# manospits/parallel_heat

Hardware: AMD Instinct MI355X
Metric: Mcells/sec (whole node) + sec/1000 iters, 8192^2 grid at 1/2/4/8 MI355X (higher is better)
Workload: dtype fp32; 1 GPU; model=heat2d 5-point Jacobi (fixed boundary), grid=8192x8192, global_batch=1, seq_len=67108864, parallelism=domain-decomp 1x1 (local), tb_depth 12, halo 12, schedule sync, converge_check=False

## Files before the change

### csrc/include/heat/kernels.hpp

```cpp
#pragma once

#include <hip/hip_runtime.h>

#include <cstdint>
#include <vector>

#include "heat/topology.hpp"

namespace heat::gpu {

struct StencilGeom {
  int64_t pitch = 0;
  int64_t gx0 = 0, gy0 = 0;
  int64_t nx = 0, ny = 0;
  float cx = 0.1f, cy = 0.1f;
  int numerics = 0;
  const unsigned* gate = nullptr;
};

namespace tbv {
enum : int {
  kRing3 = 0,
  kRing4 = 1,
  kRing2 = 2,
  kRamp = 3,
  kPipeMask = 3,
  kScalar = 4,
  kPrefetch6 = 8,
  kXcdGroups = 16,
  kAltDirection = 32,
  kFloat2 = 64,
  kForceAgePairs = 256,
  kDiagNoStore = 1024,
  kSplit = 2048,
  kDiagCachedRows = 4096,
  kNoAgePairs = 16384,
  kLinear = 32768,
  kNoLinear = 65536,
  kTile = 131072,
  kTileDpp = 262144,
  kShiftMixed = 524288,
  kDefault = kRamp | kScalar | kXcdGroups,
  kDefaultDeep = kDefault | kSplit,
};
}

constexpr int kTbMaxDepth = 8;
constexpr double kTbAgeRatio = 1.0;
constexpr double kTbSplitAgeWeights[2] = {1.7, 1.0};
constexpr double kTbLinearAgeWeights[4] = {2.0, 1.95, 1.15, 1.0};
constexpr int kTbDeepDepth = 12;
bool tb_depth_supported(int k);
int tb_strip_width(int k, int lane_cols = 4);
int tb_lane_cols(int variant);

void init_field(float* origin, const Layout& L, int64_t gx0, int64_t gy0, int64_t nx,
                int64_t ny, int mode, uint64_t seed, hipStream_t st);

void naive_step(const float* src, float* dst, const StencilGeom& g, const Box& box,
                unsigned* resid, hipStream_t st);

void lds_step(const float* src, float* dst, const StencilGeom& g, const Box& box,
              unsigned* resid, hipStream_t st);

void mfma_step(const float* src, float* dst, const StencilGeom& g, const Box& box,
               unsigned* resid, hipStream_t st);

struct TbChain {
  int passes = 1;
  unsigned* flags = nullptr;
  unsigned* done = nullptr;
  unsigned* err = nullptr;
  int max_units = 0;
  bool chained = false;
};
void tb_step(const float* src, float* dst, const StencilGeom& g, const Box* boxes, int nbox,
             int depth, unsigned* resid, hipStream_t st, int waves_target = 0, int variant = -1,
             int res_level = 0, TbChain* chain = nullptr);
struct TbResidentBuffers {
  float* base[2] = {nullptr, nullptr};
  int64_t origin = 0;
  int64_t bytes = 0;
  unsigned* flags = nullptr;
  int max_tiles = 0;
  unsigned* done = nullptr;
  unsigned* err = nullptr;
};
struct TbResidentCheck {
  int pass = 0, step = 0;
};
constexpr int kTbResidentMaxChecks = 64;
bool tb_resident_fits(const Box& box, int depth, int variant = -1);
void tb_resident_step(const float* src, float* dst, const StencilGeom& g, const Box& box,
                      int depth, int passes, const TbResidentBuffers& xb, hipStream_t st,
                      int variant = -1, const TbResidentCheck* checks = nullptr,
                      int nchecks = 0, unsigned* resids = nullptr, int64_t own_rows = 0,
                      int64_t own_cols = 0);

bool tb_mid_residual(int depth);
int tb_default_variant(int depth);
int tb_auto_variant(int depth, int64_t strip_rows_per_simd);
void tb_set_stamps(unsigned long long* buf, int64_t waves);
int tb_variant_lag(int variant);
bool tb_variant_deep(int variant);
bool tb_variant_split(int variant);
struct TbTuning {
  int variant = -1;
  int rounds = 0;
  int min_len = 0;
  int waves = 0;
  double edge_frac = 1.0;
  std::vector<double> age_weights;
  int tile_rows = 0;
  int tile_waves = 0;
  int tile_xl = -1;
  int tile_max_srps = 64;
  int nt = -1;
  int res_diag = 0;
};
TbTuning tb_tuning();
void tb_set_tuning(const TbTuning& t);
int tb_default_rounds();
int tb_resident_waves(int depth, int variant);
int tb_simd_count();
int tb_auto_waves_per_simd(int depth, int64_t strip_rows_per_simd, int max_per_simd);

void pack_box(const float* origin, int64_t pitch, const Box& box, float* buf, hipStream_t st);
constexpr int kMaxBoxCopies = 8;
struct BoxCopy {
  Box box;
  float* buf = nullptr;
};
void copy_boxes(float* origin, int64_t pitch, const BoxCopy* copies, int n, bool to_buf,
                hipStream_t st);
void unpack_box(const float* buf, float* origin, int64_t pitch, const Box& box, hipStream_t st);

struct DeviceChecksum {
  unsigned long long hash;
  double sum;
  int min_key, max_key;
  unsigned long long count;
};
void checksum_block(const float* origin, int64_t pitch, int64_t lx, int64_t ly, int64_t ox,
                    int64_t oy, int64_t ny, DeviceChecksum* out, hipStream_t st);
float checksum_key_to_float(int key);

struct DeviceGate {
  unsigned stop;
  unsigned reason;
  unsigned stop_check;
  unsigned checks;
  unsigned last_bits;
  unsigned pad[3];
};
void judge_check(unsigned* resid, DeviceGate* gate, double eps, bool mpi_compat, hipStream_t st,
                 int n = 1, int slots = 1, int stride = 0);
constexpr int kTbResidentSlots = 64;

void residual_box(const float* a, const float* b, int64_t pitch, const Box& box, unsigned* resid,
                  hipStream_t st);

}
```

### csrc/kernels/exp_register.hip

```cpp
#include "tb_exp.hpp"

namespace {
const heat::gpu::TbExpKernels* table() {
  using namespace heat::gpu;
  static const TbExpKernels k{&tbp::launch,          &tbp::occupancy,
                              &tbn::launch,          &tbn::occupancy,
                              &tbxm::launch_split,   &tbxm::occupancy_split,
                              &tbxnp::launch_split,  &tbc::occupancy_chain,
                              &tbc::launch_chain};
  return &k;
}
struct Register {
  Register() { heat_register_exp_kernels(table()); }
} reg;
}

extern "C" void heat_exp_register(void) { heat_register_exp_kernels(table()); }
```

### csrc/kernels/stencil.hip

```cpp
#include <hip/hip_runtime.h>

#include <cmath>
#include <cstdlib>
#include <cstdio>
#include <cstring>
#include <iterator>
#include <map>
#include <mutex>
#include <string>
#include <tuple>
#include <vector>

#include "heat/common.hpp"
#include "heat/init_fn.hpp"
#include "heat/kernels.hpp"
#include "tb_common.hpp"
#include "tb_exp.hpp"
#include "tb_tile.hpp"

namespace heat::gpu {
namespace {

using tbdetail::in_interior;
using tbdetail::TbArgs;
using tbdetail::TbBox;
using tbdetail::wave_max_atomic;

__global__ void init_kernel(float* base, int64_t pitch, int64_t rows, int64_t hx, int64_t hy,
                            int64_t gx0, int64_t gy0, int64_t nx, int64_t ny, int mode,
                            uint64_t seed) {
  const int64_t c = int64_t(blockIdx.x) * blockDim.x + threadIdx.x;
  if (c >= pitch) return;
  for (int64_t r = blockIdx.y; r < rows; r += gridDim.y) {
    const int64_t gx = gx0 + r - hx, gy = gy0 + c - hy;
    base[r * pitch + c] = init_value(mode, gx, gy, nx, ny, seed);
  }
}

__global__ __launch_bounds__(256) void naive_kernel(const float* __restrict__ src,
                                                    float* __restrict__ dst, StencilGeom g,
                                                    Box box, unsigned* resid) {
  const int64_t c = box.c0 + int64_t(blockIdx.x) * 64 + threadIdx.x;
  const int64_t r = box.r0 + int64_t(blockIdx.y) * 4 + threadIdx.y;
  if (tbdetail::gated(g.gate)) return;
  unsigned m = 0;
  if (r < box.r1 && c < box.c1) {
    const int64_t i = r * g.pitch + c;
    const float v = src[i];
    float out = v;
    if (in_interior(g.gx0 + r, g.nx) && in_interior(g.gy0 + c, g.ny))
      out = g.numerics == 1
                ? stencil_mpi(v, src[i - g.pitch], src[i + g.pitch], src[i - 1], src[i + 1], g.cx, g.cy)
                : stencil(v, src[i - g.pitch], src[i + g.pitch], src[i - 1], src[i + 1], g.cx, g.cy);
    dst[i] = out;
    m = __float_as_uint(fabsf(out - v));
  }
  if (resid) wave_max_atomic(m, resid);
}

__global__ void pack_kernel(const float* __restrict__ origin, int64_t pitch, Box box,
                            float* __restrict__ buf) {
  const int64_t cols = box.c1 - box.c0, n = (box.r1 - box.r0) * cols;
  for (int64_t k = int64_t(blockIdx.x) * blockDim.x + threadIdx.x; k < n;
       k += int64_t(gridDim.x) * blockDim.x) {
    const int64_t r = k / cols, c = k % cols;
    buf[k] = origin[(box.r0 + r) * pitch + box.c0 + c];
  }
}

struct BoxCopies {
  BoxCopy c[kMaxBoxCopies];
};

__global__ __launch_bounds__(128) void box_copy_kernel(float* __restrict__ origin, int64_t pitch,
                                                       BoxCopies a, int to_buf) {
  const BoxCopy& c = a.c[blockIdx.y];
  const int64_t rows = c.box.r1 - c.box.r0, cols = c.box.c1 - c.box.c0;
  for (int64_t r = blockIdx.x; r < rows; r += gridDim.x) {
    float* f = origin + (c.box.r0 + r) * pitch + c.box.c0;
    float* b = c.buf + r * cols;
    for (int64_t j = threadIdx.x; j < cols; j += blockDim.x) {
      if (to_buf) b[j] = f[j];
      else f[j] = b[j];
    }
  }
}

__global__ void unpack_kernel(const float* __restrict__ buf, float* __restrict__ origin,
                              int64_t pitch, Box box) {
  const int64_t cols = box.c1 - box.c0, n = (box.r1 - box.r0) * cols;
  for (int64_t k = int64_t(blockIdx.x) * blockDim.x + threadIdx.x; k < n;
       k += int64_t(gridDim.x) * blockDim.x) {
    const int64_t r = k / cols, c = k % cols;
    origin[(box.r0 + r) * pitch + box.c0 + c] = buf[k];
  }
}

__global__ __launch_bounds__(256) void residual_kernel(const float* __restrict__ a,
                                                       const float* __restrict__ b,
                                                       int64_t pitch, Box box, unsigned* resid) {
  const int64_t c = box.c0 + int64_t(blockIdx.x) * 64 + threadIdx.x;
  unsigned m = 0;
  if (c < box.c1)
    for (int64_t r = box.r0 + blockIdx.y * 4 + threadIdx.y; r < box.r1; r += gridDim.y * 4)
      m = max(m, __float_as_uint(fabsf(a[r * pitch + c] - b[r * pitch + c])));
  wave_max_atomic(m, resid);
}

__global__ void judge_kernel(unsigned* resids, int n, int slots, int stride, DeviceGate* gate,
                             double eps, int mpi_compat) {
  constexpr int kMax = 32;
  const int lane = threadIdx.x;
  for (int i0 = 0; i0 < n; i0 += kMax) {
    const int m = min(n - i0, kMax);
    unsigned v[kMax];
#pragma unroll
    for (int j = 0; j < kMax; ++j) v[j] = (j < m && lane < slots) ? resids[lane * stride + i0 + j] : 0u;
#pragma unroll
    for (int j = 0; j < kMax; ++j)
      if (j < m && lane < slots) resids[lane * stride + i0 + j] = 0u;
    DeviceGate gl{};
    if (lane == 0) gl = *gate;
    for (int j = 0; j < m; ++j) {
      unsigned bits = v[j];
#pragma unroll
      for (int off = 32; off >= 1; off >>= 1) bits = max(bits, unsigned(__shfl_xor(int(bits), off)));
      if (lane == 0 && gl.stop == 0u) {
        float r;
        __builtin_memcpy(&r, &bits, 4);
        const unsigned ordinal = gl.checks;
        gl.checks = ordinal + 1u;
        gl.last_bits = bits;
        unsigned why = 0u;
        if ((bits & 0x7F800000u) == 0x7F800000u) why = 2u;
        else if (mpi_compat ? double(r) <= eps : r < float(eps)) why = 1u;
        if (why) {
          gl.reason = why;
          gl.stop_check = ordinal;
          gl.stop = 1u;
        }
      }
    }
    if (lane == 0) *gate = gl;
  }
}

__device__ __forceinline__ int float_key(float f) {
  const int i = __float_as_int(f);
  return i >= 0 ? i : (i ^ 0x7FFFFFFF);
}

__global__ __launch_bounds__(256) void checksum_kernel(const float* __restrict__ origin,
                                                       int64_t pitch, int64_t lx, int64_t ly,
                                                       int64_t ox, int64_t oy, int64_t ny,
                                                       DeviceChecksum* out) {
  unsigned long long h = 0, cnt = 0;
  double sum = 0.0;
  int mn = 0x7FFFFFFF, mx = int(0x80000000);
  for (int64_t r = blockIdx.y; r < lx; r += gridDim.y) {
    const float* row = origin + r * pitch;
    const uint64_t gbase = uint64_t(ox + r) * uint64_t(ny) + uint64_t(oy);
    for (int64_t c = int64_t(blockIdx.x) * blockDim.x + threadIdx.x; c < ly;
         c += int64_t(gridDim.x) * blockDim.x) {
      const float v = row[c];
      const uint32_t bits = __float_as_uint(v);
      h += mix64((gbase + uint64_t(c)) * 0x100000001B3ull ^ bits);
      sum += double(v);
      const int k = float_key(v);
      mn = min(mn, k);
      mx = max(mx, k);
      ++cnt;
    }
  }
#pragma unroll
  for (int off = 32; off >= 1; off >>= 1) {
    h += __shfl_xor(h, off);
    cnt += __shfl_xor(cnt, off);
    sum += __shfl_xor(sum, off);
    mn = min(mn, __shfl_xor(mn, off));
    mx = max(mx, __shfl_xor(mx, off));
  }
  __shared__ unsigned long long sh_h[4], sh_c[4];
  __shared__ double sh_s[4];
  __shared__ int sh_mn[4], sh_mx[4];
  const int w = threadIdx.x >> 6;
  if ((threadIdx.x & 63) == 0) {
    sh_h[w] = h;
    sh_c[w] = cnt;
    sh_s[w] = sum;
    sh_mn[w] = mn;
    sh_mx[w] = mx;
  }
  __syncthreads();
  if (threadIdx.x == 0) {
    for (int i = 1; i < int(blockDim.x >> 6); ++i) {
      h += sh_h[i];
      cnt += sh_c[i];
      sum += sh_s[i];
      mn = min(mn, sh_mn[i]);
      mx = max(mx, sh_mx[i]);
    }
    if (cnt) {
      atomicAdd(&out->hash, h);
      atomicAdd(&out->count, cnt);
      atomicAdd(&out->sum, sum);
      atomicMin(&out->min_key, mn);
      atomicMax(&out->max_key, mx);
    }
  }
}

int grid_1d(int64_t n) { return int(std::min<int64_t>(ceil_div(n, 256), 256 * 16)); }

}

bool tb_depth_supported(int k) {
  return (k >= 1 && k <= kTbMaxDepth) || k == kTbDeepDepth;
}

int tb_strip_width(int k, int lane_cols) {
  return 64 * lane_cols - 2 * int(round_up(k, lane_cols));
}
int tb_lane_cols(int variant) { return (variant & tbv::kFloat2) ? 2 : 4; }

int tb_variant_lag(int variant) {
  const int pipe = variant & tbv::kPipeMask;
  if (pipe == tbv::kRamp && (variant & tbv::kPrefetch6)) return 4;
  switch (pipe) {
    case tbv::kRing4: return 2;
    case tbv::kRing2: return 0;
    case tbv::kRamp: return 3;
    default: return 1;
  }
}

bool tb_variant_split(int variant) {
  return (variant & tbv::kSplit) && tb_variant_deep(variant);
}

bool tb_variant_deep(int variant) {
  return (variant & tbv::kScalar) && !(variant & tbv::kFloat2) && tb_variant_lag(variant) == 3;
}

namespace {
TbTuning tuning_from_env() {
  TbTuning t;
  auto geti = [](const char* n, int def) {
    const char* e = std::getenv(n);
    return e && *e ? std::atoi(e) : def;
  };
  t.variant = geti("HEAT_TB_VARIANT", -1);
  t.rounds = std::max(0, geti("HEAT_TB_ROUNDS", 0));
  t.min_len = std::max(0, geti("HEAT_TB_MINLEN", 0));
  t.waves = std::max(0, geti("HEAT_TB_WAVES", 0));
  t.tile_rows = std::max(0, geti("HEAT_TB_TILE_ROWS", 0));
  t.tile_waves = std::max(0, geti("HEAT_TB_TILE_WAVES", 0));
  t.tile_xl = geti("HEAT_TB_TILE_XL", -1);
  t.res_diag = geti("HEAT_TB_RES_DIAG", 0) & 31;
  t.nt = geti("HEAT_TB_NT", -1);
  t.tile_max_srps = std::max(0, geti("HEAT_TB_TILE_MAX", 64));
  if (const char* e = std::getenv("HEAT_TB_EDGE_FRAC"); e && *e) t.edge_frac = std::atof(e);
  if (const char* e = std::getenv("HEAT_TB_AGE_WEIGHTS"); e && *e) {
    for (const char* q = e; *q;) {
      char* end = nullptr;
      const double v = std::strtod(q, &end);
      if (end == q) break;
      t.age_weights.push_back(v);
      q = *end == ',' ? end + 1 : end;
    }
  } else if (const char* r = std::getenv("HEAT_TB_AGE_RATIO"); r && *r) {
    t.age_weights = {std::atof(r), 1.0};
  }
  return t;
}
std::mutex g_tuning_mu;
TbTuning& tuning_ref() {
  static TbTuning t = tuning_from_env();
  return t;
}
}

TbTuning tb_tuning() {
  std::lock_guard<std::mutex> lk(g_tuning_mu);
  return tuning_ref();
}

void tb_set_tuning(const TbTuning& t) {
  std::lock_guard<std::mutex> lk(g_tuning_mu);
  tuning_ref() = t;
}

int tb_default_rounds() { return tb_tuning().rounds; }

namespace {
bool tb_trace_enabled() {
  static const bool on = [] {
    const char* e = std::getenv("HEAT_TB_TRACE");
    return e && *e && *e != '0';
  }();
  return on;
}
void tb_trace_once(const char* line) {
  static std::mutex mu;
  static std::vector<std::string> seen;
  std::lock_guard<std::mutex> lk(mu);
  for (const auto& s : seen)
    if (s == line) return;
  seen.emplace_back(line);
  std::fputs(line, stderr);
}
}

int tb_simd_count() {
  static std::map<int, int> cache;
  static std::mutex mu;
  int dev = 0;
  HIP_CHECK(hipGetDevice(&dev));
  std::lock_guard<std::mutex> lk(mu);
  auto it = cache.find(dev);
  if (it != cache.end()) return it->second;
  int cus = 0;
  HIP_CHECK(hipDeviceGetAttribute(&cus, hipDeviceAttributeMultiprocessorCount, dev));
  return cache.emplace(dev, std::max(1, cus) * 4).first->second;
}

int tb_auto_waves_per_simd(int depth, int64_t strip_rows_per_simd, int max_per_simd) {
  int w = max_per_simd;
  if (strip_rows_per_simd < 6 * int64_t(depth)) w = 1;
  else if (strip_rows_per_simd * 2 < 25 * int64_t(depth)) w = 2;
  return std::max(1, std::min(w, max_per_simd));
}

int tb_resident_waves(int depth, int variant) {
  static std::map<std::tuple<int, int, int>, int> cache;
  static std::mutex mu;
  int dev = 0;
  HIP_CHECK(hipGetDevice(&dev));
  std::lock_guard<std::mutex> lk(mu);
  auto key = std::make_tuple(dev, depth, variant);
  auto it = cache.find(key);
  if (it != cache.end()) return it->second;
  int cus = 0;
  HIP_CHECK(hipDeviceGetAttribute(&cus, hipDeviceAttributeMultiprocessorCount, dev));
  const int lag = tb_variant_lag(variant);
  if (tb_variant_split(variant)) {
    const int occ = (variant & tbv::kShiftMixed)
                        ? tb_exp("the mixed-shift split build (kShiftMixed)").tbxm_occupancy_split(depth)
                        : tbx::occupancy_split(depth);
    const int w = std::max(1, cus * std::max(1, occ) * 2);
    cache.emplace(key, w);
    return w;
  }
  const int per_cu = (variant & tbv::kFloat2)  ? tb_exp("the float2-lane build (kFloat2)").tbn_occupancy(depth, lag)
                     : (variant & tbv::kScalar) ? tbs::occupancy(depth, lag)
                                                : tb_exp("the packed build (no kScalar)").tbp_occupancy(depth, lag);
  const int w = std::max(1, cus * std::max(1, per_cu) * 4);
  cache.emplace(key, w);
  return w;
}

int tb_default_variant(int depth) {
  if (const int v = tb_tuning().variant; v >= 0) return v;
  return depth == kTbDeepDepth ? tbv::kDefaultDeep : tbv::kDefault;
}

int tb_auto_variant(int depth, int64_t strip_rows_per_simd) {
  if (const int v = tb_tuning().variant; v >= 0) return v;
  if (depth >= 4 && depth % 2 == 0 && strip_rows_per_simd < tb_tuning().tile_max_srps)
    return tbv::kTile | tbv::kXcdGroups;
  if (depth == kTbDeepDepth && strip_rows_per_simd < 64) return tbv::kDefault;
  if (depth == 8 && strip_rows_per_simd >= 256) return tbv::kDefaultDeep;
  return tb_default_variant(depth);
}

void init_field(float* origin, const Layout& L, int64_t gx0, int64_t gy0, int64_t nx, int64_t ny,
                int mode, uint64_t seed, hipStream_t st) {
  float* base = origin - L.origin();
  dim3 grid(unsigned(ceil_div(L.pitch, 256)), unsigned(std::min<int64_t>(L.rows, 1024)));
  hipLaunchKernelGGL(init_kernel, grid, dim3(256), 0, st, base, L.pitch, L.rows, int64_t(L.hx),
                     int64_t(L.hy), gx0, gy0, nx, ny, mode, seed);
  HIP_CHECK(hipGetLastError());
}

void naive_step(const float* src, float* dst, const StencilGeom& g, const Box& box,
                unsigned* resid, hipStream_t st) {
  if (box.empty()) return;
  dim3 grid(unsigned(ceil_div(box.cols(), 64)), unsigned(ceil_div(box.rows(), 4)));
  hipLaunchKernelGGL(naive_kernel, grid, dim3(64, 4), 0, st, src, dst, g, box, resid);
  HIP_CHECK(hipGetLastError());
}

namespace {
struct Stamps {
  unsigned long long* buf = nullptr;
  int64_t waves = 0;
};
std::mutex g_stamps_mu;
std::map<int, Stamps> g_stamps;

Stamps stamps_of_current_device() {
  int dev = 0;
  HIP_CHECK(hipGetDevice(&dev));
  std::lock_guard<std::mutex> lk(g_stamps_mu);
  auto it = g_stamps.find(dev);
  return it == g_stamps.end() ? Stamps{} : it->second;
}
}

void tb_set_stamps(unsigned long long* buf, int64_t waves) {
  int dev = 0;
  HIP_CHECK(hipGetDevice(&dev));
  std::lock_guard<std::mutex> lk(g_stamps_mu);
  if (buf) g_stamps[dev] = Stamps{buf, waves};
  else g_stamps.erase(dev);
}

bool tb_mid_residual(int depth) {
  return depth == kTbDeepDepth && tb_tuning().variant < 0;
}

namespace {
std::mutex g_exp_mu;
const TbExpKernels* g_exp = nullptr;
}

bool tb_exp_loaded() {
  std::lock_guard<std::mutex> lk(g_exp_mu);
  return g_exp != nullptr;
}

const TbExpKernels& tb_exp(const char* what) {
  std::lock_guard<std::mutex> lk(g_exp_mu);
  HEAT_CHECK(g_exp != nullptr,
             "%s is an experiment kernel build: `make exp`, then load "
             "parallel_heat_amd/_lib/libheat_exp.so (HEAT_EXP=1)", what);
  return *g_exp;
}

bool split_pk_enabled() {
  static const bool on = [] {
    const char* e = std::getenv("HEAT_TB_SPLIT_PK");
    return e && *e && *e != '0';
  }();
  return on;
}

constexpr int64_t kTbStreamBytes = int64_t(192) << 20;

void tb_step(const float* src, float* dst, const StencilGeom& g, const Box* boxes, int nbox,
             int depth, unsigned* resid, hipStream_t st, int waves_target, int variant,
             int res_level, TbChain* chain) {
  if (chain) chain->chained = false;
  HEAT_CHECK(nbox >= 0 && nbox <= 5, "nbox=%d", nbox);
  HEAT_CHECK(res_level >= 0 && res_level <= depth, "residual level %d of a depth-%d pass",
             res_level, depth);
  if (res_level == depth || resid == nullptr) res_level = 0;
  const bool forced = variant >= 0 || tb_tuning().variant >= 0;
  const TbTuning tune = tb_tuning();
  if (variant < 0) {
    const int W4 = tb_strip_width(depth, 4);
    int64_t rows4 = 0;
    for (int b = 0; b < nbox; ++b)
      if (!boxes[b].empty()) rows4 += ceil_div(boxes[b].cols(), W4) * boxes[b].rows();
    variant = tb_auto_variant(depth, rows4 / tb_simd_count());
    if (!tb_depth_supported(depth) && depth % 2 == 0 && depth <= 16)
      variant = tbv::kTile | tbv::kXcdGroups;
  }
  const bool tile_depth = (variant & tbv::kTile) && depth % 2 == 0 && depth <= 16;
  HEAT_CHECK(tb_depth_supported(depth) || tile_depth, "unsupported TB depth %d (variant %d)", depth,
             variant);
  if (variant & tbv::kTile) {
    if (depth % 2 == 0) {
      tbw::step(src, dst, g, boxes, nbox, depth, resid, res_level, st, variant, tune);
      return;
    }
    variant = (variant & ~(tbv::kTile | tbv::kTileDpp | 3)) | tbv::kDefault;
  }
  HEAT_CHECK(res_level == 0 || (tb_variant_split(variant) && depth == kTbDeepDepth),
             "a residual at step %d of a depth-%d pass needs the depth-12 level-split or tile "
             "kernel (variant %d%s)", res_level, depth, variant, forced ? ", forced" : "");
  const int lag = tb_variant_lag(variant);
  const int W = tb_strip_width(depth, tb_lane_cols(variant));
  int64_t total_strip_rows = 0;
  for (int b = 0; b < nbox; ++b)
    if (!boxes[b].empty()) total_strip_rows += ceil_div(boxes[b].cols(), W) * boxes[b].rows();
  const std::vector<double>& env_weights = tune.age_weights;
  const bool split_v = tb_variant_split(variant);
  int G = 0;
  std::vector<double> weights;
  auto set_weights = [&](int max_groups) {
    if (!env_weights.empty())
      weights = env_weights;
    else if (split_v)
      weights.assign(std::begin(kTbSplitAgeWeights), std::end(kTbSplitAgeWeights));
    else
      weights = {kTbAgeRatio, 1.0};
    bool uneven = false;
    for (double w : weights) uneven = uneven || w != weights[0] || w <= 0.0;
    G = uneven && int(weights.size()) >= 2 && int(weights.size()) <= max_groups ? int(weights.size()) : 0;
  };
  if (variant & tbv::kForceAgePairs) {
    set_weights(4);
    if (G == 0) {
      G = 2;
      weights.assign(2, 1.0);
    }
  }
  int bpc = 0;
  if (waves_target <= 0) {
    const int resident = tb_resident_waves(depth, variant);
    const int rounds = waves_target < 0 ? -waves_target : tune.rounds;
    if (rounds > 0) {
      waves_target = rounds * resident;
    } else {
      const int simds = tb_simd_count();
      const int per_simd = tb_auto_waves_per_simd(depth, total_strip_rows / simds,
                                                  std::max(1, resident / simds));
      waves_target = simds * per_simd;
      const int blocks_per_cu = split_v ? 2 * per_simd : per_simd;
      bpc = blocks_per_cu;
      if (G == 0 && blocks_per_cu >= 2 && !(variant & tbv::kFloat2) &&
          !(variant & tbv::kNoAgePairs))
        set_weights(blocks_per_cu);
    }
  }
  const bool pairs = G > 0;
  TbArgs args{};
  args.src = src;
  args.dst = dst;
  args.resid = resid;
  args.res_level = res_level > 0 ? res_level : depth;
  args.g = g;
  args.flags = ((variant & tbv::kXcdGroups) ? tbdetail::kTbXcdGroups : 0) |
               ((variant & tbv::kAltDirection) ? tbdetail::kTbAltDirection : 0) |
               ((variant & tbv::kDiagNoStore) ? tbdetail::kTbDiagNoStore : 0) |
               ((variant & tbv::kDiagCachedRows) ? tbdetail::kTbDiagCachedRows : 0);
  const int64_t min_len = tune.min_len > 0 ? tune.min_len : std::max<int64_t>(depth, 8);
  int64_t len = std::max<int64_t>(min_len, ceil_div(total_strip_rows, waves_target));
  const double edge_frac = tune.edge_frac;
  int n = 0, waves = 0;
  auto plan = [&](int64_t L) {
    const int64_t edge_len = std::max<int64_t>(std::min<int64_t>(min_len, L),
                                               int64_t(double(L) * edge_frac));
    n = 0;
    waves = 0;
    auto add = [&](const Box& B, int64_t clen) {
      if (B.empty()) return;
      HEAT_CHECK(n < tbdetail::kMaxBoxes, "too many TB sub-boxes");
      TbBox& t = args.box[n++];
      t.r0 = B.r0;
      t.r1 = B.r1;
      t.c0 = B.c0;
      t.c1 = B.c1;
      t.nstrips = int(ceil_div(B.cols(), W));
      t.chunk_len = int(std::min<int64_t>(clen, B.rows()));
      t.nchunks = int(ceil_div(B.rows(), t.chunk_len));
      if (pairs) {
        t.chunk_len = int(std::max<int64_t>(1, ceil_div(std::min<int64_t>(G * clen, B.rows()), G)));
        t.nchunks = int(ceil_div(B.rows(), G * int64_t(t.chunk_len)));
      }
      t.wave_begin = waves;
      waves += t.nstrips * t.nchunks * (pairs ? G : 1);
    };
    for (int b = 0; b < nbox; ++b) {
      const Box& B = boxes[b];
      if (B.empty()) continue;
      HEAT_CHECK(B.c0 % 4 == 0, "TB box column start %lld not a multiple of 4", (long long)B.c0);
      Box mid = B, top{}, bot{};
      if (edge_len < L && B.rows() > 2 * L) {
        const int64_t top_end = 1 - g.gx0 + depth;
        const int64_t bot_begin = g.nx - 2 - g.gx0 - depth;
        if (B.r0 < top_end) {
          const int64_t e = std::min(B.r1, std::max(top_end, B.r0 + edge_len));
          top = Box{B.r0, e, B.c0, B.c1};
          mid.r0 = e;
        }
        if (B.r1 - 1 > bot_begin && mid.r1 > mid.r0) {
          const int64_t s0 = std::max(mid.r0, std::min(bot_begin + 1, B.r1 - edge_len));
          bot = Box{s0, B.r1, B.c0, B.c1};
          mid.r1 = s0;
        }
      }
      add(top, edge_len);
      add(mid, L);
      add(bot, edge_len);
    }
  };
  bool linear = variant & tbv::kLinear;
  if (!linear) {
    plan(len);
    for (int it = 0; it < 8 && waves > waves_target; ++it) {
      len = std::max(len + 1, ceil_div(len * int64_t(waves), int64_t(waves_target)));
      plan(len);
    }
    linear = !(variant & tbv::kNoLinear) && waves < (9 * int64_t(waves_target)) / 10 &&
             total_strip_rows >= 32 * int64_t(depth) * waves_target;
  }
  if (linear) {
    n = 0;
    int64_t total = 0;
    for (int b = 0; b < nbox; ++b) {
      const Box& B = boxes[b];
      if (B.empty()) continue;
      HEAT_CHECK(B.c0 % 4 == 0, "TB box column start %lld not a multiple of 4", (long long)B.c0);
      TbBox& t = args.box[n++];
      t.r0 = B.r0;
      t.r1 = B.r1;
      t.c0 = B.c0;
      t.c1 = B.c1;
      t.nstrips = int(ceil_div(B.cols(), W));
      t.nchunks = 1;
      t.chunk_len = int(std::min<int64_t>(B.rows(), INT32_MAX));
      t.wave_begin = 0;
      t.lin0 = total;
      total += int64_t(t.nstrips) * B.rows();
    }
    if (n == 0) return;
    if (pairs && env_weights.empty() && split_v && bpc >= 4) {
      weights.assign(std::begin(kTbLinearAgeWeights), std::end(kTbLinearAgeWeights));
      G = int(weights.size());
    }
    const int Gl = pairs ? G : 1;
    const int64_t units = std::max<int64_t>(
        Gl, std::min<int64_t>(waves_target, total / std::max<int64_t>(1, min_len)));
    waves = int(units / Gl * Gl);
    args.lin_total = total;
    args.lin_slack = 2 * int64_t(depth);
    args.flags |= tbdetail::kTbLinear;
  }
  if (n == 0) return;
  args.nbox = n;
  args.total_waves = waves;
  if (pairs) {
    for (int b = 0; b < n; ++b) args.box[b].wave_begin /= G;
    args.total_waves = waves / G;
    args.flags |= tbdetail::kTbAgePairs;
    args.age_groups = G;
    double tot = 0.0;
    for (double w : weights) tot += w;
    double acc = 0.0;
    args.age_cum[0] = 0;
    for (int a = 0; a < G; ++a) {
      acc += weights[size_t(a)];
      args.age_cum[a + 1] = a + 1 == G ? 1024 : int(std::lround(1024.0 * acc / tot));
    }
  }
  const bool split = tb_variant_split(variant);
  if (split && !(variant & tbv::kShiftMixed)) {
    int64_t bytes = 0;
    for (int b = 0; b < nbox; ++b)
      if (!boxes[b].empty()) bytes += boxes[b].rows() * g.pitch * int64_t(sizeof(float));
    const bool nt = tune.nt >= 0 ? tune.nt != 0 : bytes > kTbStreamBytes;
    if (nt) args.flags |= tbdetail::kTbStreamRows;
  }
  if (tb_trace_enabled()) {
    char line[320];
    std::snprintf(line, sizeof line,
                  "[heat tb] depth %d variant %d boxes %d strip_rows %lld waves_target %d bpc %d "
                  "linear %d units %d age_groups %d cum %d,%d,%d,%d chunk0 %d nchunks0 %d nt %d\n",
                  depth, variant, n, (long long)total_strip_rows, waves_target, bpc,
                  int((args.flags & tbdetail::kTbLinear) != 0), waves, pairs ? G : 0,
                  args.age_cum[1], args.age_cum[2], args.age_cum[3], args.age_cum[4],
                  args.box[0].chunk_len, args.box[0].nchunks,
                  int((args.flags & tbdetail::kTbStreamRows) != 0));
    tb_trace_once(line);
  }
  if (const Stamps sb = stamps_of_current_device(); sb.buf) {
    const int64_t need = int64_t(waves) * (split ? 2 : 1);
    HEAT_CHECK(need <= sb.waves, "stamp buffer holds %lld waves, launch has %lld",
               (long long)sb.waves, (long long)need);
    args.stamps = sb.buf;
  }
  if (chain && chain->passes > 1) {
    const int G = (args.flags & tbdetail::kTbAgePairs) ? args.age_groups : 1;
    int blocks = (args.total_waves + 1) / 2;
    if (G > 1) blocks = (blocks + 7) / 8 * 8 * G;
    static const int occ = tb_exp("the chained build (HEAT_TB_CHAIN=1)").tbc_occupancy_chain(kTbDeepDepth);
    int dev = 0, cus = 0;
    HIP_CHECK(hipGetDevice(&dev));
    HIP_CHECK(hipDeviceGetAttribute(&cus, hipDeviceAttributeMultiprocessorCount, dev));
    const bool fits = split && !(variant & tbv::kShiftMixed) && (args.flags & tbdetail::kTbStreamRows) &&
                      !(args.flags & tbdetail::kTbLinear) && !(args.flags & tbdetail::kTbAltDirection) &&
                      n == 1 && resid == nullptr && depth == kTbDeepDepth && args.stamps == nullptr &&
                      int64_t(args.total_waves) * G <= chain->max_units && blocks <= cus * occ;
    if (tb_trace_enabled()) {
      char line[320];
      std::snprintf(line, sizeof line,
                    "[heat chain] passes %d split %d mixed %d stream %d linear %d alt %d boxes %d resid %d "
                    "depth %d units %d x %d max %d blocks %d cus %d occ %d -> %d\n",
                    chain->passes, int(split), int((variant & tbv::kShiftMixed) != 0),
                    int((args.flags & tbdetail::kTbStreamRows) != 0),
                    int((args.flags & tbdetail::kTbLinear) != 0),
                    int((args.flags & tbdetail::kTbAltDirection) != 0), n, int(resid != nullptr), depth,
                    args.total_waves, G, chain->max_units, blocks, cus, occ, int(fits));
      tb_trace_once(line);
    }
    if (fits) {
      chain->chained = tb_exp("the chained build (HEAT_TB_CHAIN=1)")
                           .tbc_launch_chain(args, depth, chain->passes, chain->flags, chain->done,
                                             chain->err, st);
      HIP_CHECK(hipGetLastError());
      return;
    }
  }
  bool ok;
  if (split) {
    if (variant & tbv::kShiftMixed)
      ok = tb_exp("the mixed-shift split build (kShiftMixed)").tbxm_launch_split(args, depth, st);
    else if (!(args.flags & tbdetail::kTbStreamRows))
      ok = tbx::launch_split(args, depth, st);
    else if (split_pk_enabled())
      ok = tb_exp("the packed split build (HEAT_TB_SPLIT_PK=1)").tbxnp_launch_split(args, depth, st);
    else
      ok = tbxn::launch_split(args, depth, st);
  } else if (variant & tbv::kFloat2) {
    ok = tb_exp("the float2-lane build (kFloat2)").tbn_launch(args, depth, lag, st);
  } else if (variant & tbv::kScalar) {
    ok = tbs::launch(args, depth, lag, st);
  } else {
    ok = tb_exp("the packed build (no kScalar)").tbp_launch(args, depth, lag, st);
  }
  HEAT_CHECK(ok, "TB depth %d is not instantiated for variant %d (depth %d: scalar ring-3+ramp only)",
             depth, variant, kTbDeepDepth);
  HIP_CHECK(hipGetLastError());
}

void pack_box(const float* origin, int64_t pitch, const Box& box, float* buf, hipStream_t st) {
  if (box.empty()) return;
  hipLaunchKernelGGL(pack_kernel, dim3(grid_1d(box.rows() * box.cols())), dim3(256), 0, st,
                     origin, pitch, box, buf);
  HIP_CHECK(hipGetLastError());
}

void copy_boxes(float* origin, int64_t pitch, const BoxCopy* copies, int n, bool to_buf,
                hipStream_t st) {
  HEAT_CHECK(n >= 0 && n <= kMaxBoxCopies, "copy_boxes: %d boxes", n);
  BoxCopies a{};
  int m = 0;
  int64_t rows = 0;
  for (int i = 0; i < n; ++i) {
    if (copies[i].box.empty()) continue;
    a.c[m++] = copies[i];
    rows = std::max(rows, copies[i].box.rows());
  }
  if (m == 0) return;
  dim3 grid(unsigned(std::min<int64_t>(rows, 2048)), unsigned(m));
  hipLaunchKernelGGL(box_copy_kernel, grid, dim3(128), 0, st, origin, pitch, a, int(to_buf));
  HIP_CHECK(hipGetLastError());
}

void unpack_box(const float* buf, float* origin, int64_t pitch, const Box& box, hipStream_t st) {
  if (box.empty()) return;
  hipLaunchKernelGGL(unpack_kernel, dim3(grid_1d(box.rows() * box.cols())), dim3(256), 0, st,
                     buf, origin, pitch, box);
  HIP_CHECK(hipGetLastError());
}

float checksum_key_to_float(int key) {
  const int i = key >= 0 ? key : (key ^ 0x7FFFFFFF);
  float f;
  std::memcpy(&f, &i, 4);
  return f;
}

void checksum_block(const float* origin, int64_t pitch, int64_t lx, int64_t ly, int64_t ox,
                    int64_t oy, int64_t ny, DeviceChecksum* out, hipStream_t st) {
  if (lx <= 0 || ly <= 0) return;
  const int64_t gx = std::min<int64_t>(ceil_div(ly, 256), 16);
  dim3 grid(unsigned(gx), unsigned(std::min<int64_t>(lx, std::max<int64_t>(1, 2048 / gx))));
  hipLaunchKernelGGL(checksum_kernel, grid, dim3(256), 0, st, origin, pitch, lx, ly, ox, oy, ny,
                     out);
  HIP_CHECK(hipGetLastError());
}

void judge_check(unsigned* resid, DeviceGate* gate, double eps, bool mpi_compat, hipStream_t st,
                 int n, int slots, int stride) {
  HEAT_CHECK(n >= 1 && slots >= 1 && slots <= 64 && (slots == 1 || stride >= n),
             "judge of %d checks x %d slots", n, slots);
  hipLaunchKernelGGL(judge_kernel, dim3(1), dim3(64), 0, st, resid, n, slots, stride, gate, eps,
                     int(mpi_compat));
  HIP_CHECK(hipGetLastError());
}

void residual_box(const float* a, const float* b, int64_t pitch, const Box& box, unsigned* resid,
                  hipStream_t st) {
  if (box.empty()) return;
  dim3 grid(unsigned(ceil_div(box.cols(), 64)),
            unsigned(std::min<int64_t>(ceil_div(box.rows(), 4), 1024)));
  hipLaunchKernelGGL(residual_kernel, grid, dim3(64, 4), 0, st, a, b, pitch, box, resid);
  HIP_CHECK(hipGetLastError());
}

}

extern "C" void heat_register_exp_kernels(const heat::gpu::TbExpKernels* k) {
  std::lock_guard<std::mutex> lk(heat::gpu::g_exp_mu);
  heat::gpu::g_exp = k;
}
```

### csrc/kernels/tb_common.hpp

```cpp
#pragma once

#include <hip/hip_runtime.h>

#include <type_traits>

#include "heat/init_fn.hpp"
#include "heat/kernels.hpp"

namespace heat::gpu::tbdetail {

struct TbBox {
  int64_t r0, r1, c0, c1;
  int nstrips, nchunks, chunk_len, wave_begin;
  int64_t lin0;
};

constexpr int kMaxBoxes = 16;
constexpr int kSplitRing = 8;

struct TbArgs {
  const float* src;
  float* dst;
  unsigned* resid;
  StencilGeom g;
  int nbox, total_waves;
  int flags;
  int res_level;
  int age_groups;
  int age_cum[5];
  unsigned long long* stamps;
  int64_t lin_total;
  int64_t lin_slack;
  TbBox box[kMaxBoxes];
};

__device__ __forceinline__ bool gated(const unsigned* gate) {
  return gate != nullptr && *gate != 0u;
}

constexpr int kTbXcdGroups = 1;
constexpr int kTbAltDirection = 2;
constexpr int kTbAgePairs = 4;
constexpr int kTbDiagNoStore = 8;
constexpr int kTbDiagCachedRows = 16;
constexpr int kTbLinear = 32;
constexpr int kTbStreamRows = 64;

__device__ __forceinline__ bool in_interior(int64_t g, int64_t n) { return g >= 1 && g <= n - 2; }

__device__ __forceinline__ void wave_max_atomic(unsigned m, unsigned* resid) {
#pragma unroll
  for (int off = 32; off >= 1; off >>= 1) m = max(m, unsigned(__shfl_xor(int(m), off)));
  if ((threadIdx.x & 63) == 0) atomicMax(resid, m);
}

__device__ __forceinline__ void group_max_atomic(unsigned m, unsigned* resid, unsigned* wg, int nact) {
#pragma unroll
  for (int off = 32; off >= 1; off >>= 1) m = max(m, unsigned(__shfl_xor(int(m), off)));
  if ((threadIdx.x & 63) == 0) {
    __hip_atomic_fetch_max(wg, m, __ATOMIC_RELAXED, __HIP_MEMORY_SCOPE_WORKGROUP);
    const unsigned n = __hip_atomic_fetch_add(wg + 1, 1u, __ATOMIC_ACQ_REL, __HIP_MEMORY_SCOPE_WORKGROUP);
    if (int(n) == nact - 1)
      atomicMax(resid, __hip_atomic_load(wg, __ATOMIC_ACQUIRE, __HIP_MEMORY_SCOPE_WORKGROUP));
  }
}

}

namespace heat::gpu::tbp {
bool launch(const tbdetail::TbArgs& args, int depth, int lag, hipStream_t st);
int occupancy(int depth, int lag);
}
namespace heat::gpu::tbs {
bool launch(const tbdetail::TbArgs& args, int depth, int lag, hipStream_t st);
int occupancy(int depth, int lag);
}
namespace heat::gpu::tbx {
bool launch_split(const tbdetail::TbArgs& args, int depth, hipStream_t st);
int occupancy_split(int depth);
bool launch_split_rl_a(const tbdetail::TbArgs& args, int depth, int rl, hipStream_t st);
bool launch_split_rl_b(const tbdetail::TbArgs& args, int depth, int rl, hipStream_t st);
bool launch_split_rl_c(const tbdetail::TbArgs& args, int depth, int rl, hipStream_t st);
}
namespace heat::gpu::tbc {
int occupancy_chain(int depth);
bool launch_chain(const tbdetail::TbArgs& args, int depth, int passes, unsigned* flags, unsigned* done,
                  unsigned* err, hipStream_t st);
}
namespace heat::gpu::tbxn {
bool launch_split(const tbdetail::TbArgs& args, int depth, hipStream_t st);
}
namespace heat::gpu::tbxm {
bool launch_split(const tbdetail::TbArgs& args, int depth, hipStream_t st);
int occupancy_split(int depth);
}
namespace heat::gpu::tbn {
bool launch(const tbdetail::TbArgs& args, int depth, int lag, hipStream_t st);
int occupancy(int depth, int lag);
}
```

### csrc/kernels/tb_exp.hpp

```cpp
#pragma once

#include "tb_common.hpp"

namespace heat::gpu {

struct TbExpKernels {
  bool (*tbp_launch)(const tbdetail::TbArgs&, int depth, int lag, hipStream_t st);
  int (*tbp_occupancy)(int depth, int lag);
  bool (*tbn_launch)(const tbdetail::TbArgs&, int depth, int lag, hipStream_t st);
  int (*tbn_occupancy)(int depth, int lag);
  bool (*tbxm_launch_split)(const tbdetail::TbArgs&, int depth, hipStream_t st);
  int (*tbxm_occupancy_split)(int depth);
  bool (*tbxnp_launch_split)(const tbdetail::TbArgs&, int depth, hipStream_t st);
  int (*tbc_occupancy_chain)(int depth);
  bool (*tbc_launch_chain)(const tbdetail::TbArgs&, int depth, int passes, unsigned* flags,
                           unsigned* done, unsigned* err, hipStream_t st);
};

const TbExpKernels& tb_exp(const char* what);
bool tb_exp_loaded();

namespace tbxnp {
bool launch_split(const tbdetail::TbArgs& args, int depth, hipStream_t st);
}

}

extern "C" void heat_register_exp_kernels(const heat::gpu::TbExpKernels* k);
```

### csrc/kernels/tb_split_nt.hip

```cpp
#include "tb_common.hpp"

#define HEAT_TB_NS tbxn
#define HEAT_TB_PACKED 0
#define HEAT_TB_SPLIT 1
#define HEAT_TB_BPERMUTE 1
#define HEAT_TB_SPLIT_ONLY 1
#define HEAT_TB_NTSTORE 1
#define HEAT_TB_NTLOAD 1
#include "tb_stream.inl"
```

Before: 5.211 million Mcells/s.

## Add packed DPP split build and per-build occupancy for streaming split kernel

Adds a build selector (plain, streaming non-temporal, packed/DPP) for the split temporal-blocking kernel. Resident-wave and blocks-per-CU sizing now uses the occupancy of the build actually launched. The streaming build gets launch bounds of 4 blocks per CU. Wave-target computation for split variants is reworked around resident blocks per CU. A new packed DPP kernel is added but selected only through the nt tuning knob. This trades extra complexity and register-pressure risk for higher occupancy on large grids.

New measurement: 5.217 million Mcells/s (median of 2 runs). Within noise of the previous version (+0.1%).

```diff
diff --git a/csrc/include/heat/kernels.hpp b/csrc/include/heat/kernels.hpp
--- a/csrc/include/heat/kernels.hpp
+++ b/csrc/include/heat/kernels.hpp
@@ -121,7 +121,8 @@
 TbTuning tb_tuning();
 void tb_set_tuning(const TbTuning& t);
 int tb_default_rounds();
-int tb_resident_waves(int depth, int variant);
+enum TbSplitBuild { kTbBuildPlain = 0, kTbBuildStream = 1, kTbBuildPackedDpp = 2 };
+int tb_resident_waves(int depth, int variant, int build = kTbBuildPlain);
 int tb_simd_count();
 int tb_auto_waves_per_simd(int depth, int64_t strip_rows_per_simd, int max_per_simd);
 
diff --git a/csrc/kernels/exp_register.hip b/csrc/kernels/exp_register.hip
--- a/csrc/kernels/exp_register.hip
+++ b/csrc/kernels/exp_register.hip
@@ -7,7 +7,8 @@
                               &tbn::launch,          &tbn::occupancy,
                               &tbxm::launch_split,   &tbxm::occupancy_split,
                               &tbxnp::launch_split,  &tbc::occupancy_chain,
-                              &tbc::launch_chain};
+                              &tbc::launch_chain,    &tbxd::launch_split,
+                              &tbxd::occupancy_split};
   return &k;
 }
 struct Register {
diff --git a/csrc/kernels/stencil.hip b/csrc/kernels/stencil.hip
--- a/csrc/kernels/stencil.hip
+++ b/csrc/kernels/stencil.hip
@@ -331,13 +331,14 @@
   return std::max(1, std::min(w, max_per_simd));
 }
 
-int tb_resident_waves(int depth, int variant) {
-  static std::map<std::tuple<int, int, int>, int> cache;
+int tb_resident_waves(int depth, int variant, int build) {
+  if (!tb_variant_split(variant) || (variant & tbv::kShiftMixed)) build = 0;
+  static std::map<std::tuple<int, int, int, int>, int> cache;
   static std::mutex mu;
   int dev = 0;
   HIP_CHECK(hipGetDevice(&dev));
   std::lock_guard<std::mutex> lk(mu);
-  auto key = std::make_tuple(dev, depth, variant);
+  auto key = std::make_tuple(dev, depth, variant, build);
   auto it = cache.find(key);
   if (it != cache.end()) return it->second;
   int cus = 0;
@@ -346,7 +347,10 @@
   if (tb_variant_split(variant)) {
     const int occ = (variant & tbv::kShiftMixed)
                         ? tb_exp("the mixed-shift split build (kShiftMixed)").tbxm_occupancy_split(depth)
-                        : tbx::occupancy_split(depth);
+                    : build == kTbBuildPackedDpp
+                        ? tb_exp("the packed / DPP split build (HEAT_TB_NT=2)").tbxd_occupancy_split(depth)
+                    : build == kTbBuildStream    ? tbxn::occupancy_split(depth)
+                                                 : tbx::occupancy_split(depth);
     const int w = std::max(1, cus * std::max(1, occ) * 2);
     cache.emplace(key, w);
     return w;
@@ -447,9 +451,27 @@
 
 constexpr int64_t kTbStreamBytes = int64_t(192) << 20;
 
+constexpr int kTbAutoStreamBuildClassic = kTbBuildStream;
+constexpr int kTbAutoStreamBuildLinear = kTbBuildStream;
+
+namespace {
+void tb_step_build(const float* src, float* dst, const StencilGeom& g, const Box* boxes, int nbox,
+                   int depth, unsigned* resid, hipStream_t st, int waves_target, int variant,
+                   int res_level, TbChain* chain, int nt_knob);
+}
+
 void tb_step(const float* src, float* dst, const StencilGeom& g, const Box* boxes, int nbox,
              int depth, unsigned* resid, hipStream_t st, int waves_target, int variant,
              int res_level, TbChain* chain) {
+  tb_step_build(src, dst, g, boxes, nbox, depth, resid, st, waves_target, variant, res_level, chain,
+                tb_tuning().nt);
+}
+
+namespace {
+void tb_step_build(const float* src, float* dst, const StencilGeom& g, const Box* boxes, int nbox,
+                   int depth, unsigned* resid, hipStream_t st, int waves_target, int variant,
+                   int res_level, TbChain* chain, int nt_knob) {
+  const int waves_target_in = waves_target, variant_in = variant, res_level_in = res_level;
   if (chain) chain->chained = false;
   HEAT_CHECK(nbox >= 0 && nbox <= 5, "nbox=%d", nbox);
   HEAT_CHECK(res_level >= 0 && res_level <= depth, "residual level %d of a depth-%d pass",
@@ -486,6 +508,18 @@
     if (!boxes[b].empty()) total_strip_rows += ceil_div(boxes[b].cols(), W) * boxes[b].rows();
   const std::vector<double>& env_weights = tune.age_weights;
   const bool split_v = tb_variant_split(variant);
+  int build = kTbBuildPlain;
+  if (split_v && !(variant & tbv::kShiftMixed)) {
+    int64_t bytes = 0;
+    for (int b = 0; b < nbox; ++b)
+      if (!boxes[b].empty()) bytes += boxes[b].rows() * g.pitch * int64_t(sizeof(float));
+    if (nt_knob >= 0)
+      build = std::min(nt_knob, int(kTbBuildPackedDpp));
+    else if (bytes > kTbStreamBytes)
+      build = (chain && chain->passes > 1) || res_level > 0 ? int(kTbBuildStream)
+              : (variant & tbv::kLinear)                      ? kTbAutoStreamBuildLinear
+                                                              : kTbAutoStreamBuildClassic;
+  }
   int G = 0;
   std::vector<double> weights;
   auto set_weights = [&](int max_groups) {
@@ -508,16 +542,18 @@
   }
   int bpc = 0;
   if (waves_target <= 0) {
-    const int resident = tb_resident_waves(depth, variant);
+    const int resident = tb_resident_waves(depth, variant, build);
     const int rounds = waves_target < 0 ? -waves_target : tune.rounds;
     if (rounds > 0) {
       waves_target = rounds * resident;
     } else {
       const int simds = tb_simd_count();
-      const int per_simd = tb_auto_waves_per_simd(depth, total_strip_rows / simds,
-                                                  std::max(1, resident / simds));
-      waves_target = simds * per_simd;
-      const int blocks_per_cu = split_v ? 2 * per_simd : per_simd;
+      const int res_blocks = std::max(2, resident / (simds / 2));
+      const int per_simd = tb_auto_waves_per_simd(
+          depth, total_strip_rows / simds,
+          std::max(1, split_v ? (res_blocks + 1) / 2 : resident / simds));
+      const int blocks_per_cu = split_v ? std::min(2 * per_simd, res_blocks) : per_simd;
+      waves_target = split_v ? (simds / 2) * blocks_per_cu : simds * per_simd;
       bpc = blocks_per_cu;
       if (G == 0 && blocks_per_cu >= 2 && !(variant & tbv::kFloat2) &&
           !(variant & tbv::kNoAgePairs))
@@ -596,6 +632,12 @@
     linear = !(variant & tbv::kNoLinear) && waves < (9 * int64_t(waves_target)) / 10 &&
              total_strip_rows >= 32 * int64_t(depth) * waves_target;
   }
+  if (linear && nt_knob < 0 && build != kTbBuildPlain && build != kTbAutoStreamBuildLinear &&
+      !(chain && chain->passes > 1) && res_level == 0) {
+    tb_step_build(src, dst, g, boxes, nbox, depth, resid, st, waves_target_in, variant_in, res_level_in,
+                  chain, kTbAutoStreamBuildLinear);
+    return;
+  }
   if (linear) {
     n = 0;
     int64_t total = 0;
@@ -646,23 +688,17 @@
     }
   }
   const bool split = tb_variant_split(variant);
-  if (split && !(variant & tbv::kShiftMixed)) {
-    int64_t bytes = 0;
-    for (int b = 0; b < nbox; ++b)
-      if (!boxes[b].empty()) bytes += boxes[b].rows() * g.pitch * int64_t(sizeof(float));
-    const bool nt = tune.nt >= 0 ? tune.nt != 0 : bytes > kTbStreamBytes;
-    if (nt) args.flags |= tbdetail::kTbStreamRows;
-  }
+  if (build != kTbBuildPlain) args.flags |= tbdetail::kTbStreamRows;
   if (tb_trace_enabled()) {
     char line[320];
     std::snprintf(line, sizeof line,
                   "[heat tb] depth %d variant %d boxes %d strip_rows %lld waves_target %d bpc %d "
-                  "linear %d units %d age_groups %d cum %d,%d,%d,%d chunk0 %d nchunks0 %d nt %d\n",
+                  "linear %d units %d age_groups %d cum %d,%d,%d,%d chunk0 %d nchunks0 %d nt %d build %d\n",
                   depth, variant, n, (long long)total_strip_rows, waves_target, bpc,
                   int((args.flags & tbdetail::kTbLinear) != 0), waves, pairs ? G : 0,
                   args.age_cum[1], args.age_cum[2], args.age_cum[3], args.age_cum[4],
                   args.box[0].chunk_len, args.box[0].nchunks,
-                  int((args.flags & tbdetail::kTbStreamRows) != 0));
+                  int((args.flags & tbdetail::kTbStreamRows) != 0), build);
     tb_trace_once(line);
   }
   if (const Stamps sb = stamps_of_current_device(); sb.buf) {
@@ -707,8 +743,10 @@
   if (split) {
     if (variant & tbv::kShiftMixed)
       ok = tb_exp("the mixed-shift split build (kShiftMixed)").tbxm_launch_split(args, depth, st);
-    else if (!(args.flags & tbdetail::kTbStreamRows))
+    else if (build == kTbBuildPlain)
       ok = tbx::launch_split(args, depth, st);
+    else if (build == kTbBuildPackedDpp)
+      ok = tb_exp("the packed / DPP split build (HEAT_TB_NT=2)").tbxd_launch_split(args, depth, st);
     else if (split_pk_enabled())
       ok = tb_exp("the packed split build (HEAT_TB_SPLIT_PK=1)").tbxnp_launch_split(args, depth, st);
     else
@@ -724,6 +762,7 @@
              depth, variant, kTbDeepDepth);
   HIP_CHECK(hipGetLastError());
 }
+}
 
 void pack_box(const float* origin, int64_t pitch, const Box& box, float* buf, hipStream_t st) {
   if (box.empty()) return;
diff --git a/csrc/kernels/tb_common.hpp b/csrc/kernels/tb_common.hpp
--- a/csrc/kernels/tb_common.hpp
+++ b/csrc/kernels/tb_common.hpp
@@ -89,6 +89,7 @@
 }
 namespace heat::gpu::tbxn {
 bool launch_split(const tbdetail::TbArgs& args, int depth, hipStream_t st);
+int occupancy_split(int depth);
 }
 namespace heat::gpu::tbxm {
 bool launch_split(const tbdetail::TbArgs& args, int depth, hipStream_t st);
diff --git a/csrc/kernels/tb_exp.hpp b/csrc/kernels/tb_exp.hpp
--- a/csrc/kernels/tb_exp.hpp
+++ b/csrc/kernels/tb_exp.hpp
@@ -15,6 +15,8 @@
   int (*tbc_occupancy_chain)(int depth);
   bool (*tbc_launch_chain)(const tbdetail::TbArgs&, int depth, int passes, unsigned* flags,
                            unsigned* done, unsigned* err, hipStream_t st);
+  bool (*tbxd_launch_split)(const tbdetail::TbArgs&, int depth, hipStream_t st);
+  int (*tbxd_occupancy_split)(int depth);
 };
 
 const TbExpKernels& tb_exp(const char* what);
@@ -23,6 +25,10 @@
 namespace tbxnp {
 bool launch_split(const tbdetail::TbArgs& args, int depth, hipStream_t st);
 }
+namespace tbxd {
+bool launch_split(const tbdetail::TbArgs& args, int depth, hipStream_t st);
+int occupancy_split(int depth);
+}
 
 }
 
diff --git a/csrc/kernels/tb_split_nt.hip b/csrc/kernels/tb_split_nt.hip
--- a/csrc/kernels/tb_split_nt.hip
+++ b/csrc/kernels/tb_split_nt.hip
@@ -7,4 +7,5 @@
 #define HEAT_TB_SPLIT_ONLY 1
 #define HEAT_TB_NTSTORE 1
 #define HEAT_TB_NTLOAD 1
+#define HEAT_TB_SPLIT_BLOCKS 4
 #include "tb_stream.inl"
diff --git a/csrc/kernels/tb_split_pkd.hip b/csrc/kernels/tb_split_pkd.hip
--- /dev/null
+++ b/csrc/kernels/tb_split_pkd.hip
@@ -0,0 +1,19 @@
+#include "tb_common.hpp"
+
+#define HEAT_TB_NS tbxd
+#define HEAT_TB_PACKED 1
+#define HEAT_TB_SPLIT 1
+#define HEAT_TB_BPERMUTE 0
+#define HEAT_TB_SPLIT_ONLY 1
+#define HEAT_TB_NTSTORE 1
+#define HEAT_TB_NTLOAD 1
+#ifndef HEAT_TB_SPLIT_WAVES
+#define HEAT_TB_SPLIT_WAVES 2
+#endif
+#ifndef HEAT_TB_SPLIT_BLOCKS
+#define HEAT_TB_SPLIT_BLOCKS 2
+#endif
+#ifndef HEAT_TB_PREFETCH
+#define HEAT_TB_PREFETCH 5
+#endif
+#include "tb_stream.inl"
```
